# rmcar17/SpectralClusterSupertree

Hardware: AMD Instinct MI355X
Metric: top-level PCG build + Fiedler solve wall-time (s) at N taxa, 1/2/4/8 MI355X (lower is better)
Workload: dtype f64 (loop operator: fp32 image of W; fp64 renewal + confirmation)

## Files before the change

### spectralclustersupertree_amd/csrc/scs_build.hip

```cpp

#include <algorithm>

#include "scs_internal.h"

typedef unsigned long long u64;
typedef unsigned int u32;

constexpr u32 DEPTH_INF = 0xFFFFFFFFu;


__device__ __forceinline__ void rmq_offsets(int m, int a, int b, int (&o)[2]) {
    const int k = 31 - __clz(b - a);
    o[0] = k * m + a;
    o[1] = k * m + b - (1 << k);
}

template <typename K>
__device__ __forceinline__ K rmq_min(const K *__restrict__ base, int m, int a, int b) {
    int o[2];
    rmq_offsets(m, a, b, o);
    const K x = base[o[0]], y = base[o[1]];
    return x < y ? x : y;
}

// ... 391 lines not shown
};

struct ev_pair {
    hipEvent_t a = nullptr, b = nullptr;
    ~ev_pair() {
        if (a) hipEventDestroy(a);
        if (b) hipEventDestroy(b);
    }
    int init() {
        SCS_HIP_CHECK(hipEventCreate(&a));
        SCS_HIP_CHECK(hipEventCreate(&b));
        return SCS_OK;
    }
};

int levels_for(int64_t m) {
    int l = 0;
    while (((int64_t)1 << l) <= m) ++l;
    return l;
}

}

static int graph_alloc(scs_ctx *ctx, int32_t n, int32_t row_begin, int32_t row_end,
                       hipStream_t stream, scs_graph **out, int32_t col0 = 0) {
    auto *g = new scs_graph();
    g->n = n;
    g->row_begin = row_begin;
    g->row_end = row_end;
    g->col0 = col0;
    g->upper = col0 > 0 || false;
    g->ld = scs_round_up(n - col0, SCS_LD_ALIGN);
    const size_t rows = (size_t)(row_end - row_begin);
    size_t bytes = rows * (size_t)g->ld * sizeof(double);
    if (bytes < 16) bytes = 16;
    {
        const int rc = scs_block_alloc(ctx, bytes, (void **)&g->d_w);
        if (rc != SCS_OK) {
            delete g;
            return rc;
        }
        g->w_bytes = bytes;
        g->w_block = true;
    }
    if (g->ld > n - col0) {
        hipError_t e = hipMemset2DAsync(g->d_w + (n - col0), (size_t)g->ld * 8, 0,
                                        (size_t)(g->ld - (n - col0)) * 8, rows, stream);
        if (e != hipSuccess) {
            if (g->w_block) scs_block_release(ctx, g->d_w);
            else scs_dev_free(g->d_w);
            delete g;
            scs_set_error("cannot clear the padding of W: %s", hipGetErrorString(e));
            return SCS_EHIP;
        }
    }
    *out = g;
    return SCS_OK;
}

extern "C" int scs_graph_free(scs_ctx *ctx, scs_graph *g) {
    if (!g) return SCS_OK;
    if (ctx) hipSetDevice(ctx->device);
    if (g->mf) {
        if (ctx) hipStreamSynchronize(ctx->stream);
        scs_matfree_release(g);
    }
    if (ctx && g->d_w && g->w_block) {
        scs_block_release(ctx, g->d_w);
    } else if (ctx && g->d_w) {
        if (!ctx->w_cache || g->w_bytes >= ctx->w_cache_bytes) {
// ... 141 lines not shown
            k_block_records_wide<PIPE_NG><<<grid_r, 64, 0, s>>>(tb->d_tree_off, b.t0, tl0, b.nb, b.pos, b.npad, b.st_off, st,
                                                          b.am_off, b.am, b.row_begin, b.row_end, b.rec);
        else if (b.kind == PREP_MONO)
            k_block_records_mono<<<grid_r, 64, 0, s>>>(tb->d_tree_off, b.t0, tl0, b.nb, b.pos, b.npad, b.st_off, st,
                                                       b.am_off, b.am, b.row_begin, b.row_end, b.rec);
    } else {
        gap_entry *st = (gap_entry *)b.st;
        k_positions_pairs<<<grid_l, 256, 0, s>>>(tb->d_tree_off, tb->d_leaf_taxon, tb->d_adj_depth, tb->d_adj_val,
                                                 tb->d_tree_w, b.t0, tl0, b.pos, b.npad, b.st_off, st);
        if (fused)
            k_sparse_levels_fused<gap_entry><<<(unsigned)np, 1024, 0, s>>>(tb->d_tree_off, b.t0, tl0, b.st_off, st,
                                                                           b.am_off, b.am, pick_shallower_pair{});
        else
            for (int k = 1; k < max_levels; ++k)
                k_sparse_level<gap_entry><<<grid_l, 256, 0, s>>>(tb->d_tree_off, b.t0, tl0, k, b.st_off, st, b.am_off,
                                                                 b.am, pick_shallower_pair{});
        k_block_records_gen<<<grid_r, 64, 0, s>>>(tb->d_tree_off, b.t0, tl0, b.nb, b.pos, b.npad, b.st_off, st, b.am_off,
                                                  b.am, b.row_begin, b.row_end, b.rec);
    }
    SCS_HIP_CHECK(hipGetLastError());
    return SCS_OK;
}

struct pinned_ref {
    scs_ctx *ctx;
    hipStream_t stream;
    void *p = nullptr;
    bool in_flight = false;
    pinned_ref(scs_ctx *c, hipStream_t s) : ctx(c), stream(s) {}
    ~pinned_ref() {
        if (!p) return;
        if (in_flight) hipStreamSynchronize(stream);
        scs_pinned_release(ctx, p);
    }
};

}

extern "C" int scs_pcg_build(scs_ctx *ctx, const scs_tables *tb, int32_t row_begin,
                             int32_t row_end, int32_t flags, scs_graph **out,
                             scs_build_stats *stats) {
    SCS_REQUIRE(ctx && tb && out, "scs_pcg_build: null argument");
    SCS_REQUIRE((flags & ~(SCS_BUILD_MONOTONE | SCS_BUILD_SHARED | SCS_BUILD_UPPER | SCS_BUILD_SCATTER)) == 0,
                "scs_pcg_build: unknown flag bits 0x%x", flags);
    const bool scatter = (flags & SCS_BUILD_SCATTER) != 0;
    if (scatter && tb) SCS_TRY(scs_tables_finish(ctx, tb));
// ... 19 lines not shown
    static_assert(MONO_TCW == SCS_TCW, "one tile width for all kernels");
    const size_t entry_bytes = monotone ? 8 : sizeof(gap_entry);
    size_t rec_bytes = monotone ? R3_BYTES : G3_BYTES;
    const int n_cgroups = (n + cols_per_tile - 1) / cols_per_tile;
    const int64_t npad = scs_round_up((int64_t)n_cgroups * cols_per_tile, SCS_NPAD);
    bool shared = (flags & SCS_BUILD_SHARED) != 0 && world > 1;
    if (shared) {
        const int64_t nb_all = (n + SCS_TR - 1) / SCS_TR;
        const double tile_bytes = 0.5 * (double)nb_all * n_cgroups * SCS_TR * cols_per_tile * 8.0;
        if (tile_bytes * (1.0 + 1.0 / world) > 96.0 * 1024 * 1024 * 1024) shared = false;
    }
    const int b_row_begin = shared ? 0 : row_begin, b_row_end = shared ? n : row_end;
    const bool sym = !shared && (row_begin == 0 && row_end == n && world == 1);
    const bool trapezoid = (flags & SCS_BUILD_UPPER) != 0;
    if (trapezoid)
        SCS_REQUIRE(row_begin % cols_per_tile == 0,
                    "scs_pcg_build: SCS_BUILD_UPPER needs row_begin (%d) to be a multiple of %d", row_begin,
                    cols_per_tile);
    const bool upper = sym || shared || trapezoid;
    const int gb0 = b_row_begin / SCS_TR;
    const int rows = row_end - row_begin;
    const int n_blocks = (b_row_end - b_row_begin + SCS_TR - 1) / SCS_TR;

    scs_graph *g = nullptr;
    SCS_TRY(graph_alloc(ctx, n, row_begin, row_end, s, &g, trapezoid ? row_begin : 0));
    g->upper = trapezoid;
    if (scatter) SCS_HIP_CHECK(hipMemsetAsync(g->d_w, 0, (size_t)rows * (size_t)g->ld * 8, s));
    double *w_base = g->d_w - g->col0;
    struct guard {
        scs_ctx *c;
        scs_graph *g;
        ~guard() {
            if (g) scs_graph_free(c, g);
        }
    } gd{ctx, g};

    std::vector<int2> tiles;
    tiles.reserve((size_t)n_blocks * n_cgroups);
    for (int b = 0; b < n_blocks; ++b)
        for (int c = 0; c < n_cgroups; ++c) {
            if (upper && (int64_t)(c + 1) * cols_per_tile <= (int64_t)(gb0 + b) * SCS_TR) continue;
            tiles.push_back(make_int2(b, c));
        }
    {
        const bool per_xcd = !(scs_dbg("SCS_TILE_ORDER") && atoi(scs_dbg("SCS_TILE_ORDER")) == 0);
        auto xcd_reorder = [](std::vector<int2> &v) {
            if (v.size() <= 8) return;
            std::vector<int2> per[8];
            for (const int2 &t : v) per[t.x & 7].push_back(t);
            std::vector<int2> ordered;
            ordered.reserve(v.size());
            size_t at[8] = {0, 0, 0, 0, 0, 0, 0, 0};
            while (ordered.size() < v.size())
                for (int x = 0; x < 8; ++x)
                    if (at[x] < per[x].size()) ordered.push_back(per[x][at[x]++]);
            v.swap(ordered);
        };
        if (per_xcd && !shared) {
            xcd_reorder(tiles);
        } else if (per_xcd) {
            std::vector<std::vector<int2>> share(world);
            for (size_t i = 0; i < tiles.size(); ++i) share[i % world].push_back(tiles[i]);
            for (auto &v : share) xcd_reorder(v);
            for (int r = 0; r < world; ++r)
                for (size_t k = 0; k < share[r].size(); ++k) tiles[(size_t)world * k + r] = share[r][k];
        }
    }
    std::vector<int2> all_tiles;
    dev_buf d_all_tiles(ctx);
    cached_buf d_tile_out(ctx), d_gathered(ctx);
    size_t chunk_doubles = 0;
    const bool exchange_allgather =
        scs_dbg("SCS_EXCHANGE") && std::string(scs_dbg("SCS_EXCHANGE")) == "allgather";
    if (shared) {
        all_tiles.swap(tiles);
        for (size_t i = rank; i < all_tiles.size(); i += world) tiles.push_back(all_tiles[i]);
        const size_t slots = (all_tiles.size() + world - 1) / world;
        chunk_doubles = slots * SCS_TR * cols_per_tile;
        SCS_TRY(d_all_tiles.alloc(all_tiles.size() * sizeof(int2)));
        SCS_HIP_CHECK(hipMemcpyAsync(d_all_tiles.p, all_tiles.data(),
                                     all_tiles.size() * sizeof(int2), hipMemcpyHostToDevice, s));
        SCS_TRY(d_tile_out.alloc(chunk_doubles * 8));
        if (exchange_allgather) SCS_TRY(d_gathered.alloc(chunk_doubles * 8 * world));
        if (tiles.size() < slots)
            SCS_HIP_CHECK(hipMemsetAsync((double *)d_tile_out.p + (slots - 1) * SCS_TR * cols_per_tile,
                                         0, (size_t)SCS_TR * cols_per_tile * 8, s));
    }
    pooled_buf d_tiles(ctx, 0);
    SCS_TRY(d_tiles.alloc(std::max<size_t>(tiles.size(), 1) * sizeof(int2)));
    SCS_HIP_CHECK(hipMemcpyAsync(d_tiles.p, tiles.data(), tiles.size() * sizeof(int2),
                                 hipMemcpyHostToDevice, s));

    bool tree_par = sym && !scatter && !tiles.empty() && tiles.size() <= 24 && tb->n_trees >= 128;
    if (const char *e = scs_dbg("SCS_TREE_PARALLEL")) tree_par = sym && !scatter && !tiles.empty() && atoi(e) != 0;
    const size_t cells_per_tree = tiles.size() * (size_t)SCS_TR * cols_per_tile * 8;

    const size_t wide_min_tiles = 13;
    bool listed = monotone && !scatter && !tiles.empty() && tb->n_trees > 0 &&
                  (double)tb->n_leaves / ((double)tb->n_trees * std::max(n, 1)) < 1.0 / 64.0;
    if (const char *e = scs_dbg("SCS_TILE_LISTS")) listed = monotone && !scatter && !tiles.empty() && atoi(e) != 0;
    if (listed) tree_par = false;
    int wide_mode = (monotone && !scatter && !tree_par && !listed && tiles.size() >= wide_min_tiles) ? 3 : 0;
    bool wide_forced = false;
    if (const char *e = scs_dbg("SCS_WIDE")) {
        wide_mode = (monotone && !scatter && !tiles.empty() && atoi(e)) ? 3 : 0;
        wide_forced = wide_mode != 0;
        if (wide_mode) listed = false;
    }
    if (wide_mode && ctx->max_lds_bytes < (int)spec_layout::LDS_BYTES) {
        wide_mode = 0;
        wide_forced = false;
    }
    if (wide_mode) tree_par = false;
    const bool wide = wide_mode != 0;
    const int group_tiles = PIPE_NG;
    std::vector<int4> groups;
    dev_buf d_groups(ctx);
    if (wide) {
        rec_bytes = wide_layout<PIPE_NG>::BYTES;
        std::vector<std::vector<int>> of_block((size_t)n_blocks);
        for (size_t i = 0; i < tiles.size(); ++i) of_block[(size_t)tiles[i].x].push_back((int)i);
        std::vector<int4> per[8];
        for (int b = 0; b < n_blocks; ++b) {
            const std::vector<int> &v = of_block[(size_t)b];
            for (size_t k = 0; k < v.size(); k += group_tiles)
                per[b & 7].push_back(make_int4(v[k], k + 1 < v.size() ? v[k + 1] : -1,
                                               (group_tiles > 2 && k + 2 < v.size()) ? v[k + 2] : -1, 0));
        }
        size_t total = 0, at[8] = {0, 0, 0, 0, 0, 0, 0, 0};
        for (auto &v : per) total += v.size();
        groups.reserve(total);
        while (groups.size() < total)
            for (int x = 0; x < 8; ++x)
                if (at[x] < per[x].size()) groups.push_back(per[x][at[x]++]);
        SCS_TRY(d_groups.alloc(groups.size() * sizeof(int4)));
        SCS_HIP_CHECK(hipMemcpyAsync(d_groups.p, groups.data(), groups.size() * sizeof(int4),
                                     hipMemcpyHostToDevice, s));
    }

    const int M = tb->n_trees;
    std::vector<int> batch_start{0};
    {
        const int batch_trees_env = scs_dbg("SCS_BATCH_TREES") ? atoi(scs_dbg("SCS_BATCH_TREES")) : 0;
        int max_batch_trees = 256;
        {
            const double avg_leaves = (double)tb->n_leaves / std::max(M, 1);
            const double table_bytes =
                (double)table_entries((int64_t)std::max(avg_leaves - 1.0, 1.0)) * (double)entry_bytes;
            max_batch_trees = (int)std::min(256.0, std::max(64.0, 600e6 / std::max(table_bytes, 1.0)));
        }
        if (n <= 2048) max_batch_trees = 4096;
        const int arrived = tb->late_start.empty() ? M : tb->late_start[0];
        if (wide) {
            const int rest = M - (arrived < M ? arrived : 0);
            const int k = std::max(1, (rest + 511) / 512);
            max_batch_trees = std::max(96, (rest + k - 1) / k);
        }
        if (tree_par)
            max_batch_trees = (int)std::max<size_t>(16, std::min<size_t>((size_t)max_batch_trees,
                                                                         SCS_SCRATCH_KEEP / cells_per_tree));
        if (batch_trees_env > 0) max_batch_trees = batch_trees_env;
        if (tree_par)
            max_batch_trees = (int)std::max<size_t>(1, std::min<size_t>((size_t)max_batch_trees,
                                                                        SCS_SCRATCH_KEEP / std::max<size_t>(cells_per_tree, 1)));
        size_t used = 0;
        for (int t = 0; t < M; ++t) {
            const int64_t nt = tb->h_tree_off[t + 1] - tb->h_tree_off[t];
            const int64_t m = nt - 1;
            const size_t need = (size_t)table_entries(m) * entry_bytes + (size_t)argmin_entries(m) * sizeof(argmin_t) +
                                (size_t)npad * 4 + (size_t)n_blocks * rec_bytes;
            if ((used + need > ctx->ws_limit || t - batch_start.back() >= max_batch_trees ||
                 (t == arrived && batch_start.size() == 1)) &&
                t > batch_start.back()) {
                batch_start.push_back(t);
                used = 0;
            }
            used += need;
        }
        batch_start.push_back(M);
    }
    const int n_batches = (int)batch_start.size() - 1;

    struct ev_ref {
        hipEvent_t a, b;
    } ev_total, ev_prep, ev_acc;
    for (auto &e : ctx->build_events)
        if (!e) SCS_HIP_CHECK(hipEventCreate(&e));
    ev_total = {ctx->build_events[0], ctx->build_events[1]};
    ev_prep = {ctx->build_events[2], ctx->build_events[3]};
    ev_acc = {ctx->build_events[4], ctx->build_events[5]};
    float prep_ms = 0.f, acc_ms = 0.f;
    SCS_HIP_CHECK(hipEventRecord(ev_total.a, s));

    int spec_batches = 0, spec_trees = 0;
    float spec_ms = 0.f;
    bool single_batch_spec = false;
    pooled_buf d_pos(ctx, 1), d_am(ctx, 2), d_st(ctx, 3), d_stoff(ctx, 4), d_rec(ctx, 5), d_cells(ctx, 6);
    dev_buf d_pcol(ctx), d_lists(ctx), d_list_cnt(ctx);
    int listed_batches = 0;
    std::vector<size_t> off_at((size_t)n_batches + 1, 0);
    for (int bi = 0; bi < n_batches; ++bi)
        off_at[bi + 1] = off_at[bi] + 2 * (size_t)(batch_start[bi + 1] - batch_start[bi] + 1);
    pinned_ref h_off(ctx, s);
    SCS_TRY(scs_pinned_get(ctx, std::max<size_t>(off_at[n_batches], 2) * 8, &h_off.p));
    {
        int64_t *h = (int64_t *)h_off.p;
        for (int bi = 0; bi < n_batches; ++bi) {
            const int t0 = batch_start[bi], nb = batch_start[bi + 1] - t0;
            int64_t *st_off = h + off_at[bi], *am_off = st_off + nb + 1;
            st_off[0] = am_off[0] = 0;
            for (int t = 0; t < nb; ++t) {
                const int64_t m = tb->h_tree_off[t0 + t + 1] - tb->h_tree_off[t0 + t] - 1;
                st_off[t + 1] = st_off[t] + table_entries(m);
                am_off[t + 1] = am_off[t] + argmin_entries(m);
            }
        }
        SCS_TRY(d_stoff.alloc(off_at[n_batches] * 8));
        h_off.in_flight = true;
        SCS_HIP_CHECK(hipMemcpyAsync(d_stoff.p, h, off_at[n_batches] * 8, hipMemcpyHostToDevice, s));
    }
    const bool by_arrival = !(scs_dbg("SCS_PREP_BY_ARRIVAL") && atoi(scs_dbg("SCS_PREP_BY_ARRIVAL")) == 0);
    int prep_pieces = 0;
    for (int bi = 0; bi < n_batches; ++bi) {
        const int t0 = batch_start[bi], t1 = batch_start[bi + 1];
        const int nb = t1 - t0;
        const int64_t *h_st_off = (const int64_t *)h_off.p + off_at[bi], *h_am_off = h_st_off + nb + 1;
        int64_t max_n = 0;
        for (int t = t0; t < t1; ++t) max_n = std::max(max_n, tb->h_tree_off[t + 1] - tb->h_tree_off[t]);
        const size_t need_pos = (size_t)nb * npad * 4;
        const size_t need_st = (size_t)h_st_off[nb] * entry_bytes + 64;
        const size_t need_am = (size_t)h_am_off[nb] * sizeof(argmin_t) + 64;
        const size_t need_rec = (size_t)n_blocks * nb * rec_bytes;
        const int wide_min_trees = wide_forced ? 1 : 96;
        const bool wide_b = wide && (nb >= wide_min_trees || (groups.size() >= 8 * 256 && nb >= 16));
        if (wide_b) {
            ++spec_batches;
            spec_trees += nb;
            single_batch_spec = true;
        }
        SCS_TRY(d_pos.alloc(need_pos));
        SCS_TRY(d_st.alloc(need_st));
        SCS_TRY(d_am.alloc(need_am));
        SCS_TRY(d_rec.alloc(need_rec));

        SCS_HIP_CHECK(hipEventRecord(ev_prep.a, s));
        SCS_HIP_CHECK(hipMemsetAsync(d_pos.p, 0xFF, need_pos, s));
        prep_batch pb;
        pb.tb = tb;
        pb.t0 = t0;
        pb.nb = nb;
        pb.kind = !monotone ? PREP_GEN : wide_b ? PREP_WIDE : scatter ? PREP_NO_RECORDS : PREP_MONO;
        pb.pos = (int32_t *)d_pos.p;
        pb.npad = npad;
        pb.st_off = (const int64_t *)d_stoff.p + off_at[bi];
        pb.am_off = pb.st_off + nb + 1;
        pb.st = d_st.p;
        pb.am = (argmin_t *)d_am.p;
        pb.rec = (unsigned char *)d_rec.p;
        pb.n_blocks = n_blocks;
        pb.row_begin = b_row_begin;
        pb.row_end = b_row_end;
        for (int p0 = t0; p0 < t1;) {
            int p1 = t1;
            if (by_arrival)
                for (const int32_t c : tb->late_start)
                    if (c > p0 && c < p1) p1 = c;
            SCS_TRY(scs_tables_wait(ctx, tb, p1, s));
            SCS_TRY(prep_piece(pb, p0 - t0, p1 - p0, s));
            ++prep_pieces;
            p0 = p1;
        }
        SCS_HIP_CHECK(hipEventRecord(ev_prep.b, s));

        SCS_HIP_CHECK(hipEventRecord(ev_acc.a, s));
        const unsigned nt = (unsigned)tiles.size();
        if (scatter) {
            const int64_t nbk = (max_n + 63) / 64;
            k_scatter_atomic<<<dim3((unsigned)(nbk * (nbk + 1) / 2), (unsigned)nb), 256, 0, s>>>(
                tb->d_tree_off, tb->d_leaf_taxon, t0, pb.st_off, (const double *)d_st.p,
                g->d_w, g->ld);
        } else if (monotone) {
            mono_params mp;
            mp.tiles = (const int2 *)d_tiles.p;
            mp.rec = (const unsigned char *)d_rec.p;
            mp.pos = (const int32_t *)d_pos.p;
            mp.npad = npad;
            mp.stv = (const double *)d_st.p;
            mp.n_batch = nb;
            mp.w = w_base;
            mp.ld = g->ld;
            mp.n = n;
            mp.row_begin = b_row_begin;
            mp.row_end = b_row_end;
            mp.load_w = bi > 0;
            mp.mirror = (sym && bi == n_batches - 1) ? 1 : 0;
            mp.tile_out = shared ? (double *)d_tile_out.p : nullptr;
            mp.stamps = nullptr;
            mp.split_tiles = 0;
            mp.lists = nullptr;
            mp.list_cnt = nullptr;
            const bool stamp = scs_dbg("SCS_ACC_STAMP") && atoi(scs_dbg("SCS_ACC_STAMP"));
            if (wide_b) {
                wide_params wp;
                wp.m = mp;
                wp.groups = (const int4 *)d_groups.p;
                wp.producer_prio = 2;
                const unsigned ng = (unsigned)groups.size();
                dev_buf d_st8(ctx);
                if (stamp) {
                    SCS_TRY(d_st8.alloc(64));
                    SCS_HIP_CHECK(hipMemsetAsync(d_st8.p, 0, 64, s));
                    wp.m.stamps = (unsigned long long *)d_st8.p;
                }
#define SCS_LAUNCH_SPEC(SYM_, STAMP_)                                                                   \
    do {                                                                                                \
        SCS_HIP_CHECK(hipFuncSetAttribute((const void *)k_accumulate_spec<SYM_, STAMP_>,                \
                                          hipFuncAttributeMaxDynamicSharedMemorySize,                   \
                                          (int)spec_layout::LDS_BYTES));                                \
        k_accumulate_spec<SYM_, STAMP_><<<ng, spec_layout::THREADS, spec_layout::LDS_BYTES, s>>>(wp);   \
    } while (0)
                if (ng) {
                    if (stamp && sym) SCS_LAUNCH_SPEC(true, true);
                    else if (stamp) SCS_LAUNCH_SPEC(false, true);
                    else if (sym) SCS_LAUNCH_SPEC(true, false);
                    else SCS_LAUNCH_SPEC(false, false);
                }
#undef SCS_LAUNCH_SPEC
                if (stamp) {
// ... 21 lines not shown
                const char *nm[7] = {"wait loads+record", "barrier A", "combine", "search + issue",
                                     "expand", "barrier B", "cells"};
                double tot = 0;
                for (int i = 0; i < 7; ++i) tot += (double)h[i];
                for (int i = 0; i < 7; ++i)
                    fprintf(stderr, "[stamp] %-24s %6.2f %%  (%.0f cycles per wave-step)\n", nm[i],
                            100.0 * h[i] / tot, (double)h[i] / ((double)h[7] * nb));
            } else if (nt && tree_par) {
                SCS_TRY(d_cells.alloc((size_t)nb * cells_per_tree));
                mono_params ap = mp;
                ap.split_tiles = (int)nt;
                ap.load_w = 0;
                ap.mirror = 0;
                ap.tile_out = (double *)d_cells.p;
                k_accumulate_mono<true, false><<<nt * (unsigned)nb, MONO_TCW, 0, s>>>(ap);
                k_sum_tree_tiles<true, mono_params><<<nt * SCS_TR, MONO_TCW, 0, s>>>(mp, (const double *)d_cells.p,
                                                                                    (int)nt);
            } else if (nt && listed) {
                SCS_TRY(d_pcol.alloc((size_t)n_cgroups * nb));
                SCS_TRY(d_lists.alloc((size_t)nt * nb * 4));
                SCS_TRY(d_list_cnt.alloc((size_t)nt * 4));
                k_col_presence<<<dim3((unsigned)n_cgroups, (unsigned)nb), 64, 0, s>>>(
                    (const int32_t *)d_pos.p, npad, n, cols_per_tile, nb, (unsigned char *)d_pcol.p);
                k_tile_lists<<<(nt + 255) / 256, 256, 0, s>>>((const int2 *)d_tiles.p, (int)nt,
                                                             (const unsigned char *)d_rec.p, R3_BYTES, R3_CNT, nb,
                                                             (const unsigned char *)d_pcol.p, (int32_t *)d_lists.p,
                                                             (int32_t *)d_list_cnt.p);
                mp.lists = (const int32_t *)d_lists.p;
                mp.list_cnt = (const int32_t *)d_list_cnt.p;
                if (sym) k_accumulate_mono<true, false, true><<<nt, MONO_TCW, 0, s>>>(mp);
                else k_accumulate_mono<false, false, true><<<nt, MONO_TCW, 0, s>>>(mp);
                ++listed_batches;
            } else if (nt) {
                if (sym) k_accumulate_mono<true, false><<<nt, MONO_TCW, 0, s>>>(mp);
                else k_accumulate_mono<false, false><<<nt, MONO_TCW, 0, s>>>(mp);
            }
        } else {
            gen_params gp;
            gp.tiles = (const int2 *)d_tiles.p;
            gp.rec = (const unsigned char *)d_rec.p;
            gp.pos = (const int32_t *)d_pos.p;
            gp.npad = npad;
            gp.ste = (const gap_entry *)d_st.p;
            gp.n_batch = nb;
            gp.w = w_base;
            gp.ld = g->ld;
            gp.n = n;
            gp.row_begin = b_row_begin;
            gp.row_end = b_row_end;
            gp.load_w = bi > 0;
            gp.mirror = (sym && bi == n_batches - 1) ? 1 : 0;
            gp.tile_out = shared ? (double *)d_tile_out.p : nullptr;
            gp.split_tiles = 0;
            if (nt && tree_par) {
                SCS_TRY(d_cells.alloc((size_t)nb * cells_per_tree));
                gen_params ap = gp;
                ap.split_tiles = (int)nt;
                ap.load_w = 0;
                ap.mirror = 0;
                ap.tile_out = (double *)d_cells.p;
                k_accumulate_gen<true><<<nt * (unsigned)nb, MONO_TCW, 0, s>>>(ap);
                k_sum_tree_tiles<true, gen_params><<<nt * SCS_TR, MONO_TCW, 0, s>>>(gp, (const double *)d_cells.p,
                                                                                   (int)nt);
            } else if (nt) {
                if (sym) k_accumulate_gen<true><<<nt, MONO_TCW, 0, s>>>(gp);
                else k_accumulate_gen<false><<<nt, MONO_TCW, 0, s>>>(gp);
            }
        }
        SCS_HIP_CHECK(hipGetLastError());
        SCS_HIP_CHECK(hipEventRecord(ev_acc.b, s));
        if (n_batches > 1) {
            SCS_HIP_CHECK(hipEventSynchronize(ev_acc.b));
            float ms = 0.f;
            SCS_HIP_CHECK(hipEventElapsedTime(&ms, ev_prep.a, ev_prep.b));
            prep_ms += ms;
            SCS_HIP_CHECK(hipEventElapsedTime(&ms, ev_acc.a, ev_acc.b));
            acc_ms += ms;
            if (wide_b) spec_ms += ms;
        }
    }
    float exch_ms = 0.f;
    double exch_bytes = 0.0;
    if (shared && exchange_allgather) {
        ev_pair ev_x;
        SCS_TRY(ev_x.init());
        SCS_HIP_CHECK(hipEventRecord(ev_x.a, s));
        SCS_TRY(scs_comm_allgather_f64(&ctx->comm, (const double *)d_tile_out.p,
                                       (double *)d_gathered.p, chunk_doubles, s));
        k_unpack_tiles<<<(unsigned)all_tiles.size(), cols_per_tile, 0, s>>>(
            (const double *)d_gathered.p, (const int2 *)d_all_tiles.p, world,
            (int64_t)chunk_doubles, n, row_begin, row_end, g->d_w, g->ld);
        SCS_HIP_CHECK(hipGetLastError());
        SCS_HIP_CHECK(hipEventRecord(ev_x.b, s));
        SCS_HIP_CHECK(hipEventSynchronize(ev_x.b));
        SCS_HIP_CHECK(hipEventElapsedTime(&exch_ms, ev_x.a, ev_x.b));
        exch_bytes = (double)chunk_doubles * 8.0 * (world - 1);
    } else if (shared) {
        std::vector<int32_t> splits;
        SCS_TRY(scs_gather_row_splits(ctx, row_begin, row_end, n, splits));
        auto needs = [&](int dst, const int2 &t) {
            const int64_t lo = splits[dst], hi = splits[dst + 1];
            const int64_t r_lo = (int64_t)t.x * SCS_TR, r_hi = std::min<int64_t>(r_lo + SCS_TR, n);
            const int64_t c_lo = (int64_t)t.y * cols_per_tile, c_hi = std::min<int64_t>(c_lo + cols_per_tile, n);
            return (r_lo < hi && lo < r_hi) || (c_lo < hi && lo < c_hi);
        };
        std::vector<int64_t> send_off(world + 1, 0), recv_off(world + 1, 0);
        std::vector<int32_t> send_slots;
        std::vector<int2> recv_tiles;
        for (int p = 0; p < world; ++p) {
            for (size_t i = rank; i < all_tiles.size(); i += world)
                if (needs(p, all_tiles[i])) send_slots.push_back((int32_t)(i / world));
            send_off[p + 1] = (int64_t)send_slots.size() * SCS_TR * cols_per_tile;
            for (size_t i = p; i < all_tiles.size(); i += world)
// ... 15 lines not shown
                                     hipMemcpyHostToDevice, s));
        if (!send_slots.empty())
            k_pack_tiles<<<(unsigned)send_slots.size(), 256, 0, s>>>(
                (const double *)d_tile_out.p, (const int32_t *)d_slots.p, cols_per_tile, (double *)d_send.p);
        SCS_HIP_CHECK(hipGetLastError());
        SCS_TRY(scs_comm_alltoallv_f64(&ctx->comm, (const double *)d_send.p, send_off.data(),
                                       (double *)d_recv.p, recv_off.data(), s));
        if (!recv_tiles.empty())
            k_unpack_received<<<(unsigned)recv_tiles.size(), cols_per_tile, 0, s>>>(
                (const double *)d_recv.p, (const int2 *)d_rtiles.p, n, row_begin, row_end, g->d_w,
                g->ld);
        SCS_HIP_CHECK(hipGetLastError());
        SCS_HIP_CHECK(hipEventRecord(ev_x.b, s));
        SCS_HIP_CHECK(hipEventSynchronize(ev_x.b));
        SCS_HIP_CHECK(hipEventElapsedTime(&exch_ms, ev_x.a, ev_x.b));
        exch_bytes = (double)(recv_off[world] - (recv_off[rank + 1] - recv_off[rank])) * 8.0;
    }
    SCS_HIP_CHECK(hipEventRecord(ev_total.b, s));
    SCS_HIP_CHECK(hipEventSynchronize(ev_total.b));
    h_off.in_flight = false;
    SCS_TRY(scs_tables_finish(ctx, tb));
    float total_ms = 0.f;
    SCS_HIP_CHECK(hipEventElapsedTime(&total_ms, ev_total.a, ev_total.b));
    if (n_batches == 1) {
        SCS_HIP_CHECK(hipEventElapsedTime(&prep_ms, ev_prep.a, ev_prep.b));
        SCS_HIP_CHECK(hipEventElapsedTime(&acc_ms, ev_acc.a, ev_acc.b));
        if (single_batch_spec) spec_ms = acc_ms;
    }

    if (stats) {
        memset(stats, 0, sizeof(*stats));
        stats->n_taxa = n;
        stats->n_trees = M;
        stats->row_begin = row_begin;
        stats->row_end = row_end;
        stats->symmetric = shared ? 2 : (sym ? 1 : 0);
        stats->exchange_ms = exch_ms;
        stats->exchange_bytes = exch_bytes;
        stats->n_tiles = (int32_t)tiles.size();
        stats->n_batches = n_batches;
        stats->spec_batches = spec_batches;
        stats->tree_parallel_batches = tree_par ? n_batches : 0;
        stats->spec_trees = spec_trees;
        stats->listed_batches = listed_batches;
        stats->prep_pieces = prep_pieces;
        stats->spec_ms = spec_ms;
        stats->cell_trees = (double)tiles.size() * SCS_TR * cols_per_tile * (double)M;
        stats->prep_ms = prep_ms;
        stats->accumulate_ms = acc_ms;
        stats->total_ms = total_ms;
// ... 343 lines not shown
```

### spectralclustersupertree_amd/csrc/scs_ctx.hip

```cpp

#include <dlfcn.h>

#include <atomic>
#include <condition_variable>
#include <mutex>

#include "scs_internal.h"
#include "scs_arena.h"

#include <chrono>
#include <pthread.h>

#include <algorithm>
#include <cmath>

static thread_local std::string g_last_error;

void scs_set_error(const char *fmt, ...) {
    char buf[1024];
    va_list ap;
    va_start(ap, fmt);
    vsnprintf(buf, sizeof(buf), fmt, ap);
    va_end(ap);
    g_last_error = buf;
// ... 1070 lines not shown
    t->max_leaves = (int32_t)max_leaves;
    t->h_tree_off.assign(tree_off, tree_off + n_trees + 1);
    t->d_block = block;
    char *base = (char *)block;
    t->d_tree_off = (int64_t *)(base + o_off);
    t->d_leaf_taxon = (int32_t *)(base + o_tax);
    t->d_adj_depth = (int32_t *)(base + o_dep);
    t->d_adj_val = (double *)(base + o_val);
    t->d_tree_w = (double *)(base + o_w);
    unsigned *d_flags = (unsigned *)(base + o_flag);
    t->d_flags = d_flags;
    hipStream_t s = ctx->stream;
    int32_t first = n_trees, chunk = n_trees;
    if (n_taxa > 2048 && (size_t)L * 16 >= ((size_t)8 << 20) && scs_is_pinned(leaf_taxon) &&
        scs_is_pinned(adj_depth) && scs_is_pinned(adj_val)) {
        const double avg = std::max((double)L / n_trees - 1.0, 1.0);
        const double table_bytes = (std::floor(std::log2(avg)) + 1.0) * avg * 8.0;
        const int32_t per = (int32_t)std::min(256.0, std::max(64.0, 600e6 / table_bytes));
        if (n_trees >= 2 * per || n_trees - per >= 32) {
            first = std::min(per, 64);
            chunk = per;
        }
    }
    const int64_t L0 = tree_off[first];
    hipError_t e = hipMemsetAsync(d_flags, 0, 4, s);
    if (e == hipSuccess) e = hipMemcpyAsync(t->d_tree_off, tree_off, ((size_t)n_trees + 1) * 8, hipMemcpyHostToDevice, s);
    if (e == hipSuccess && L0) e = hipMemcpyAsync(t->d_leaf_taxon, leaf_taxon, (size_t)L0 * 4, hipMemcpyHostToDevice, s);
    if (e == hipSuccess && L0) e = hipMemcpyAsync(t->d_adj_depth, adj_depth, (size_t)L0 * 4, hipMemcpyHostToDevice, s);
    if (e == hipSuccess && L0) e = hipMemcpyAsync(t->d_adj_val, adj_val, (size_t)L0 * 8, hipMemcpyHostToDevice, s);
    if (e == hipSuccess) e = hipMemcpyAsync(t->d_tree_w, tree_w, (size_t)n_trees * 8, hipMemcpyHostToDevice, s);
    if (e == hipSuccess) {
        const int grid = (int)std::min<int64_t>((L0 + 255) / 256 + 1, 4096);
        k_validate_tables<<<grid, 256, 0, s>>>(t->d_leaf_taxon, t->d_adj_depth, L0, n_taxa, d_flags);
        e = hipGetLastError();
    }
    if (e == hipSuccess) e = hipMemcpyAsync(ctx->h_flags, d_flags, 4, hipMemcpyDeviceToHost, s);
    if (e == hipSuccess) e = hipStreamSynchronize(s);
    if (e == hipSuccess && first < n_trees) {
        if (!ctx->copy_stream) e = hipStreamCreateWithFlags(&ctx->copy_stream, hipStreamNonBlocking);
        hipStream_t cs = ctx->copy_stream;
        for (int32_t a = first; a < n_trees && e == hipSuccess; a += chunk) {
            const int32_t b = std::min(n_trees, a + chunk);
            const int64_t p0 = tree_off[a], cnt = tree_off[b] - tree_off[a];
            e = hipMemcpyAsync(t->d_leaf_taxon + p0, leaf_taxon + p0, (size_t)cnt * 4, hipMemcpyHostToDevice, cs);
            if (e == hipSuccess) e = hipMemcpyAsync(t->d_adj_depth + p0, adj_depth + p0, (size_t)cnt * 4, hipMemcpyHostToDevice, cs);
            if (e == hipSuccess) e = hipMemcpyAsync(t->d_adj_val + p0, adj_val + p0, (size_t)cnt * 8, hipMemcpyHostToDevice, cs);
            hipEvent_t ev = nullptr;
            if (e == hipSuccess) e = hipEventCreateWithFlags(&ev, hipEventDisableTiming);
            if (e == hipSuccess) e = hipEventRecord(ev, cs);
            if (e == hipSuccess) {
                t->late_start.push_back(a);
                t->late_ev.push_back(ev);
            } else if (ev) {
                hipEventDestroy(ev);
            }
            if (e == hipSuccess) {
                const int grid = (int)std::min<int64_t>((cnt + 255) / 256 + 1, 4096);
                k_validate_tables<<<grid, 256, 0, cs>>>(t->d_leaf_taxon + p0, t->d_adj_depth + p0, cnt, n_taxa, d_flags);
                e = hipGetLastError();
            }
        }
    }
    if (e != hipSuccess) {
        scs_tables_free(ctx, t);
        scs_set_error("table upload failed: %s", hipGetErrorString(e));
        return e == hipErrorOutOfMemory ? SCS_ENOMEM : SCS_EHIP;
    }
    const unsigned bad = *ctx->h_flags;
    if (bad) {
        scs_tables_free(ctx, t);
        scs_set_error("scs_tables_upload: %s", (bad & 1u) ? "a leaf_taxon entry is out of range [0, n_taxa)"
                                                          : "an adj_depth entry is negative");
        return SCS_EINVAL;
    }
    *out = t;
    return SCS_OK;
}
```

### spectralclustersupertree_amd/csrc/scs_internal.h

```cpp
#pragma once

#include <hip/hip_runtime.h>

#include <cstdarg>
#include <cstdint>
#include <cstdio>
#include <cstring>
#include <mutex>
#include <string>
#include <vector>

#include "../../include/scs_hip.h"

void scs_set_error(const char *fmt, ...);

#define SCS_HIP_CHECK(expr)                                                                  \
    do {                                                                                     \
        hipError_t e_ = (expr);                                                              \
        if (e_ != hipSuccess) {                                                              \
            scs_set_error("%s failed: %s (%s:%d)", #expr, hipGetErrorString(e_), __FILE__,   \
                          __LINE__);                                                         \
            return (e_ == hipErrorOutOfMemory) ? SCS_ENOMEM : SCS_EHIP;                      \
        }                                                                                    \
    } while (0)
// ... 17 lines not shown
    static const bool on = [] {
        const char *e = getenv("SCS_DEBUG");
        return e && atoi(e) != 0;
    }();
    return on ? getenv(name) : nullptr;
}

struct scs_ctx;
hipError_t scs_dev_malloc_impl(scs_ctx *ctx, void **p, size_t bytes);
hipError_t scs_dev_free(void *p);
template <typename T>
static inline hipError_t scs_dev_malloc(scs_ctx *ctx, T **p, size_t bytes) {
    return scs_dev_malloc_impl(ctx, (void **)p, bytes);
}
size_t scs_arena_free_bytes(int device);

constexpr int SCS_TR = 64;
constexpr int SCS_TCW = 256;
constexpr int SCS_NPAD = 512;
constexpr int SCS_LD_ALIGN = 512;

constexpr size_t SCS_SCRATCH_KEEP = (size_t)1 << 30;
constexpr size_t SCS_PINNED_KEEP = (size_t)2 << 30;

struct scs_ctx;
int scs_block_alloc(scs_ctx *ctx, size_t bytes, void **out);
void scs_block_release(scs_ctx *ctx, void *p);
void scs_block_drop_free(scs_ctx *ctx);
int scs_pinned_get(scs_ctx *ctx, size_t bytes, void **out);
void scs_pinned_release(scs_ctx *ctx, void *p);

struct scs_local_group;

struct scs_comm {
    int rank = 0;
    int world = 1;
    int kind = 0;
    void *rccl_comm = nullptr;
    scs_local_group *group = nullptr;
};

int scs_comm_allgather_f64(scs_comm *comm, const double *sendbuf, double *recvbuf, size_t count,
                           hipStream_t stream);
int scs_comm_alltoallv_f64(scs_comm *comm, const double *sendbuf, const int64_t *send_off,
                           double *recvbuf, const int64_t *recv_off, hipStream_t stream);
int scs_comm_init_rccl(scs_comm *comm, int rank, int world, const void *uid);
// ... 40 lines not shown
        size_t o_to = 0, o_lt = 0, o_ad = 0, o_av = 0, o_tw = 0;
        int64_t n_toff = 0, n_leaf = 0, n_tree = 0;
        unsigned char *scratch = nullptr;
        size_t scratch_cap = 0;
    };
    std::vector<small_slot> small_slots;
    hipStream_t small_stream = nullptr;
};

struct scs_tables {
    int32_t n_taxa = 0;
    int32_t n_trees = 0;
    int64_t n_leaves = 0;
    int32_t max_leaves = 0;
    std::vector<int64_t> h_tree_off;
    void *d_block = nullptr;
    int64_t *d_tree_off = nullptr;
    int32_t *d_leaf_taxon = nullptr;
    int32_t *d_adj_depth = nullptr;
    double *d_adj_val = nullptr;
    double *d_tree_w = nullptr;
    mutable std::vector<int32_t> late_start;
    mutable std::vector<hipEvent_t> late_ev;
    unsigned *d_flags = nullptr;
};

int scs_tables_wait(scs_ctx *ctx, const scs_tables *t, int32_t t_end, hipStream_t stream);
int scs_tables_finish(scs_ctx *ctx, const scs_tables *t);

struct mf_data {
    const scs_tables *tb = nullptr;
    int64_t *d_stack_off = nullptr;
    int64_t stack_total = 0;
    int b_cap = 0;
    int chunks = 1;
    double *st_val = nullptr, *st_sum = nullptr;
    int32_t *st_dep = nullptr;
    double *sm_val = nullptr, *sm_sum = nullptr, *cy_pa = nullptr, *cy_ps = nullptr;
    int32_t *sm_dep = nullptr, *cy_dep = nullptr, *sm_cnt = nullptr, *sm_root = nullptr, *cy_cnt = nullptr;
    double *x = nullptr;
    double *y = nullptr;
    double *slabs = nullptr;
    int slabs_b = 0;
    int64_t n_apply = 0;
    std::vector<int32_t> maxd;
};
// ... 72 lines not shown
```

Baseline: 0.01385.

## Cut host-side sync and setup overhead in PCG build and table upload

Several host-overhead changes go in together. The tile, group and offset arrays are packed into one pinned block and sent in a single copy. The per-batch hipEventSynchronize is dropped in favour of per-batch event pairs that are read only at the end. W allocation moves after host planning, and its 2D pad memset becomes a small kernel. Table upload now sends a small first piece and streams the rest on the copy stream without a blocking sync, validating it in one pass. The aim is to remove host stalls and extra API calls; it adds more events, more complex upload ordering, and a later validation error report.

```diff
diff --git a/spectralclustersupertree_amd/csrc/scs_build.hip b/spectralclustersupertree_amd/csrc/scs_build.hip
--- a/spectralclustersupertree_amd/csrc/scs_build.hip
+++ b/spectralclustersupertree_amd/csrc/scs_build.hip
@@ -1,5 +1,6 @@
 
 #include <algorithm>
+#include <chrono>
 
 #include "scs_internal.h"
 
@@ -437,6 +438,14 @@
 
 }
 
+__global__ __launch_bounds__(256) void k_zero_pads(double *__restrict__ w, int64_t ld, int used, int padw,
+                                                   int64_t rows) {
+    const int64_t i = (int64_t)blockIdx.x * 256 + threadIdx.x;
+    if (i >= rows * padw) return;
+    const int64_t r = i / padw;
+    w[r * ld + used + (int)(i - r * padw)] = 0.0;
+}
+
 static int graph_alloc(scs_ctx *ctx, int32_t n, int32_t row_begin, int32_t row_end,
                        hipStream_t stream, scs_graph **out, int32_t col0 = 0) {
     auto *g = new scs_graph();
@@ -458,9 +467,11 @@
         g->w_bytes = bytes;
         g->w_block = true;
     }
-    if (g->ld > n - col0) {
-        hipError_t e = hipMemset2DAsync(g->d_w + (n - col0), (size_t)g->ld * 8, 0,
-                                        (size_t)(g->ld - (n - col0)) * 8, rows, stream);
+    if (g->ld > n - col0 && rows > 0) {
+        const int padw = (int)(g->ld - (n - col0));
+        const int64_t cells = (int64_t)rows * padw;
+        k_zero_pads<<<(unsigned)((cells + 255) / 256), 256, 0, stream>>>(g->d_w, g->ld, n - col0, padw, (int64_t)rows);
+        hipError_t e = hipGetLastError();
         if (e != hipSuccess) {
             if (g->w_block) scs_block_release(ctx, g->d_w);
             else scs_dev_free(g->d_w);
@@ -648,6 +659,25 @@
     return SCS_OK;
 }
 
+template <typename T, typename KEY>
+void deal_to_xcds(std::vector<T> &v, KEY key) {
+    size_t start[9] = {0, 0, 0, 0, 0, 0, 0, 0, 0};
+    for (const T &t : v) ++start[key(t) + 1];
+    size_t longest = 0;
+    for (int x = 0; x < 8; ++x) {
+        longest = std::max(longest, start[x + 1]);
+        start[x + 1] += start[x];
+    }
+    std::vector<T> sorted(v.size());
+    size_t at[8];
+    for (int x = 0; x < 8; ++x) at[x] = start[x];
+    for (const T &t : v) sorted[at[key(t)]++] = t;
+    size_t o = 0;
+    for (size_t r = 0; r < longest; ++r)
+        for (int x = 0; x < 8; ++x)
+            if (start[x] + r < start[x + 1]) v[o++] = sorted[start[x] + r];
+}
+
 struct pinned_ref {
     scs_ctx *ctx;
     hipStream_t stream;
@@ -713,18 +743,12 @@
     const int rows = row_end - row_begin;
     const int n_blocks = (b_row_end - b_row_begin + SCS_TR - 1) / SCS_TR;
 
-    scs_graph *g = nullptr;
-    SCS_TRY(graph_alloc(ctx, n, row_begin, row_end, s, &g, trapezoid ? row_begin : 0));
-    g->upper = trapezoid;
-    if (scatter) SCS_HIP_CHECK(hipMemsetAsync(g->d_w, 0, (size_t)rows * (size_t)g->ld * 8, s));
-    double *w_base = g->d_w - g->col0;
-    struct guard {
-        scs_ctx *c;
-        scs_graph *g;
-        ~guard() {
-            if (g) scs_graph_free(c, g);
-        }
-    } gd{ctx, g};
+    const bool stamps_on = scs_dbg("SCS_BUILD_STAMPS") && atoi(scs_dbg("SCS_BUILD_STAMPS"));
+    std::vector<std::pair<const char *, std::chrono::steady_clock::time_point>> host_stamps;
+    auto host_stamp = [&](const char *what) {
+        if (stamps_on) host_stamps.emplace_back(what, std::chrono::steady_clock::now());
+    };
+    host_stamp("entry");
 
     std::vector<int2> tiles;
     tiles.reserve((size_t)n_blocks * n_cgroups);
@@ -737,15 +761,7 @@
         const bool per_xcd = !(scs_dbg("SCS_TILE_ORDER") && atoi(scs_dbg("SCS_TILE_ORDER")) == 0);
         auto xcd_reorder = [](std::vector<int2> &v) {
             if (v.size() <= 8) return;
-            std::vector<int2> per[8];
-            for (const int2 &t : v) per[t.x & 7].push_back(t);
-            std::vector<int2> ordered;
-            ordered.reserve(v.size());
-            size_t at[8] = {0, 0, 0, 0, 0, 0, 0, 0};
-            while (ordered.size() < v.size())
-                for (int x = 0; x < 8; ++x)
-                    if (at[x] < per[x].size()) ordered.push_back(per[x][at[x]++]);
-            v.swap(ordered);
+            deal_to_xcds(v, [](const int2 &t) { return t.x & 7; });
         };
         if (per_xcd && !shared) {
             xcd_reorder(tiles);
@@ -758,8 +774,8 @@
         }
     }
     std::vector<int2> all_tiles;
-    dev_buf d_all_tiles(ctx);
     cached_buf d_tile_out(ctx), d_gathered(ctx);
+    bool clear_last_slot = false;
     size_t chunk_doubles = 0;
     const bool exchange_allgather =
         scs_dbg("SCS_EXCHANGE") && std::string(scs_dbg("SCS_EXCHANGE")) == "allgather";
@@ -768,19 +784,10 @@
         for (size_t i = rank; i < all_tiles.size(); i += world) tiles.push_back(all_tiles[i]);
         const size_t slots = (all_tiles.size() + world - 1) / world;
         chunk_doubles = slots * SCS_TR * cols_per_tile;
-        SCS_TRY(d_all_tiles.alloc(all_tiles.size() * sizeof(int2)));
-        SCS_HIP_CHECK(hipMemcpyAsync(d_all_tiles.p, all_tiles.data(),
-                                     all_tiles.size() * sizeof(int2), hipMemcpyHostToDevice, s));
         SCS_TRY(d_tile_out.alloc(chunk_doubles * 8));
         if (exchange_allgather) SCS_TRY(d_gathered.alloc(chunk_doubles * 8 * world));
-        if (tiles.size() < slots)
-            SCS_HIP_CHECK(hipMemsetAsync((double *)d_tile_out.p + (slots - 1) * SCS_TR * cols_per_tile,
-                                         0, (size_t)SCS_TR * cols_per_tile * 8, s));
-    }
-    pooled_buf d_tiles(ctx, 0);
-    SCS_TRY(d_tiles.alloc(std::max<size_t>(tiles.size(), 1) * sizeof(int2)));
-    SCS_HIP_CHECK(hipMemcpyAsync(d_tiles.p, tiles.data(), tiles.size() * sizeof(int2),
-                                 hipMemcpyHostToDevice, s));
+        clear_last_slot = tiles.size() < slots;
+    }
 
     bool tree_par = sym && !scatter && !tiles.empty() && tiles.size() <= 24 && tb->n_trees >= 128;
     if (const char *e = scs_dbg("SCS_TREE_PARALLEL")) tree_par = sym && !scatter && !tiles.empty() && atoi(e) != 0;
@@ -806,28 +813,28 @@
     const bool wide = wide_mode != 0;
     const int group_tiles = PIPE_NG;
     std::vector<int4> groups;
-    dev_buf d_groups(ctx);
     if (wide) {
         rec_bytes = wide_layout<PIPE_NG>::BYTES;
-        std::vector<std::vector<int>> of_block((size_t)n_blocks);
-        for (size_t i = 0; i < tiles.size(); ++i) of_block[(size_t)tiles[i].x].push_back((int)i);
-        std::vector<int4> per[8];
+        std::vector<size_t> of_start((size_t)n_blocks + 1, 0);
+        for (const int2 &t : tiles) ++of_start[(size_t)t.x + 1];
+        for (int b = 0; b < n_blocks; ++b) of_start[(size_t)b + 1] += of_start[(size_t)b];
+        std::vector<int> of_tile(tiles.size());
+        {
+            std::vector<size_t> at(of_start.begin(), of_start.end() - 1);
+            for (size_t i = 0; i < tiles.size(); ++i) of_tile[at[(size_t)tiles[i].x]++] = (int)i;
+        }
+        groups.reserve(tiles.size() / group_tiles + (size_t)n_blocks);
         for (int b = 0; b < n_blocks; ++b) {
-            const std::vector<int> &v = of_block[(size_t)b];
-            for (size_t k = 0; k < v.size(); k += group_tiles)
-                per[b & 7].push_back(make_int4(v[k], k + 1 < v.size() ? v[k + 1] : -1,
-                                               (group_tiles > 2 && k + 2 < v.size()) ? v[k + 2] : -1, 0));
-        }
-        size_t total = 0, at[8] = {0, 0, 0, 0, 0, 0, 0, 0};
-        for (auto &v : per) total += v.size();
-        groups.reserve(total);
-        while (groups.size() < total)
-            for (int x = 0; x < 8; ++x)
-                if (at[x] < per[x].size()) groups.push_back(per[x][at[x]++]);
-        SCS_TRY(d_groups.alloc(groups.size() * sizeof(int4)));
-        SCS_HIP_CHECK(hipMemcpyAsync(d_groups.p, groups.data(), groups.size() * sizeof(int4),
-                                     hipMemcpyHostToDevice, s));
-    }
+            const int *v = of_tile.data() + of_start[(size_t)b];
+            const size_t nv = of_start[(size_t)b + 1] - of_start[(size_t)b];
+            for (size_t k = 0; k < nv; k += group_tiles)
+                groups.push_back(make_int4(v[k], k + 1 < nv ? v[k + 1] : -1,
+                                           (group_tiles > 2 && k + 2 < nv) ? v[k + 2] : -1, b));
+        }
+        deal_to_xcds(groups, [](const int4 &g4) { return g4.w & 7; });
+        for (int4 &g4 : groups) g4.w = 0;
+    }
+    host_stamp("tile list and groups");
 
     const int M = tb->n_trees;
     std::vector<int> batch_start{0};
@@ -841,7 +848,7 @@
             max_batch_trees = (int)std::min(256.0, std::max(64.0, 600e6 / std::max(table_bytes, 1.0)));
         }
         if (n <= 2048) max_batch_trees = 4096;
-        const int arrived = tb->late_start.empty() ? M : tb->late_start[0];
+        const int arrived = tb->late_start.empty() ? M : std::min<int>(M, std::max<int>(tb->first_batch, tb->late_start[0]));
         if (wide) {
             const int rest = M - (arrived < M ? arrived : 0);
             const int k = std::max(1, (rest + 511) / 512);
@@ -874,28 +881,53 @@
 
     struct ev_ref {
         hipEvent_t a, b;
-    } ev_total, ev_prep, ev_acc;
+    } ev_total;
     for (auto &e : ctx->build_events)
         if (!e) SCS_HIP_CHECK(hipEventCreate(&e));
     ev_total = {ctx->build_events[0], ctx->build_events[1]};
-    ev_prep = {ctx->build_events[2], ctx->build_events[3]};
-    ev_acc = {ctx->build_events[4], ctx->build_events[5]};
+    struct batch_events {
+        scs_ctx *c;
+        std::vector<hipEvent_t> ev;
+        std::vector<char> is_spec;
+        ~batch_events() {
+            for (size_t i = 4; i < ev.size(); ++i) c->event_pool.push_back(ev[i]);
+        }
+    } bev{ctx, {}, {}};
+    bev.ev.assign(ctx->build_events + 2, ctx->build_events + 6);
+    bev.ev.reserve(4 * (size_t)n_batches);
+    while (bev.ev.size() < 4 * (size_t)n_batches) {
+        hipEvent_t e = nullptr;
+        if (!ctx->event_pool.empty()) {
+            e = ctx->event_pool.back();
+            ctx->event_pool.pop_back();
+        } else {
+            SCS_HIP_CHECK(hipEventCreate(&e));
+        }
+        bev.ev.push_back(e);
+    }
+    bev.is_spec.assign((size_t)n_batches, 0);
     float prep_ms = 0.f, acc_ms = 0.f;
-    SCS_HIP_CHECK(hipEventRecord(ev_total.a, s));
 
     int spec_batches = 0, spec_trees = 0;
     float spec_ms = 0.f;
-    bool single_batch_spec = false;
     pooled_buf d_pos(ctx, 1), d_am(ctx, 2), d_st(ctx, 3), d_stoff(ctx, 4), d_rec(ctx, 5), d_cells(ctx, 6);
     dev_buf d_pcol(ctx), d_lists(ctx), d_list_cnt(ctx);
     int listed_batches = 0;
     std::vector<size_t> off_at((size_t)n_batches + 1, 0);
     for (int bi = 0; bi < n_batches; ++bi)
         off_at[bi + 1] = off_at[bi] + 2 * (size_t)(batch_start[bi + 1] - batch_start[bi] + 1);
+    auto up256 = [](size_t b) { return (b + 255) / 256 * 256; };
+    const size_t o_tiles = up256(std::max<size_t>(off_at[n_batches], 2) * 8);
+    const size_t o_groups = o_tiles + up256(std::max<size_t>(tiles.size(), 1) * sizeof(int2));
+    const size_t o_all = o_groups + up256(groups.size() * sizeof(int4));
+    const size_t setup_bytes = o_all + up256(all_tiles.size() * sizeof(int2));
     pinned_ref h_off(ctx, s);
-    SCS_TRY(scs_pinned_get(ctx, std::max<size_t>(off_at[n_batches], 2) * 8, &h_off.p));
+    SCS_TRY(scs_pinned_get(ctx, setup_bytes, &h_off.p));
     {
         int64_t *h = (int64_t *)h_off.p;
+        if (!tiles.empty()) memcpy((char *)h_off.p + o_tiles, tiles.data(), tiles.size() * sizeof(int2));
+        if (!groups.empty()) memcpy((char *)h_off.p + o_groups, groups.data(), groups.size() * sizeof(int4));
+        if (!all_tiles.empty()) memcpy((char *)h_off.p + o_all, all_tiles.data(), all_tiles.size() * sizeof(int2));
         for (int bi = 0; bi < n_batches; ++bi) {
             const int t0 = batch_start[bi], nb = batch_start[bi + 1] - t0;
             int64_t *st_off = h + off_at[bi], *am_off = st_off + nb + 1;
@@ -906,11 +938,38 @@
                 am_off[t + 1] = am_off[t] + argmin_entries(m);
             }
         }
-        SCS_TRY(d_stoff.alloc(off_at[n_batches] * 8));
-        h_off.in_flight = true;
-        SCS_HIP_CHECK(hipMemcpyAsync(d_stoff.p, h, off_at[n_batches] * 8, hipMemcpyHostToDevice, s));
-    }
+    }
+    host_stamp("batch plan, offsets, set-up block");
+
+    scs_graph *g = nullptr;
+    SCS_TRY(graph_alloc(ctx, n, row_begin, row_end, s, &g, trapezoid ? row_begin : 0));
+    g->upper = trapezoid;
+    struct guard {
+        scs_ctx *c;
+        scs_graph *g;
+        ~guard() {
+            if (g) scs_graph_free(c, g);
+        }
+    } gd{ctx, g};
+    host_stamp("W block and its padding kernel");
+    if (scatter) SCS_HIP_CHECK(hipMemsetAsync(g->d_w, 0, (size_t)rows * (size_t)g->ld * 8, s));
+    double *w_base = g->d_w - g->col0;
+    if (clear_last_slot) {
+        const size_t slots = (all_tiles.size() + world - 1) / world;
+        SCS_HIP_CHECK(hipMemsetAsync((double *)d_tile_out.p + (slots - 1) * SCS_TR * cols_per_tile, 0,
+                                     (size_t)SCS_TR * cols_per_tile * 8, s));
+    }
+    SCS_HIP_CHECK(hipEventRecord(ev_total.a, s));
+    SCS_TRY(d_stoff.alloc(setup_bytes));
+    h_off.in_flight = true;
+    SCS_HIP_CHECK(hipMemcpyAsync(d_stoff.p, h_off.p, setup_bytes, hipMemcpyHostToDevice, s));
+    const int2 *d_tiles = (const int2 *)((const char *)d_stoff.p + o_tiles);
+    const int4 *d_groups = (const int4 *)((const char *)d_stoff.p + o_groups);
+    const int2 *d_all_tiles = (const int2 *)((const char *)d_stoff.p + o_all);
+    host_stamp("set-up copy queued");
     const bool by_arrival = !(scs_dbg("SCS_PREP_BY_ARRIVAL") && atoi(scs_dbg("SCS_PREP_BY_ARRIVAL")) == 0);
+    const bool cut_first_piece = scs_dbg("SCS_PREP_FIRST_PIECE") && atoi(scs_dbg("SCS_PREP_FIRST_PIECE"));
+    const int32_t no_cut_below = (tb->late_start.empty() || cut_first_piece) ? 0 : tb->first_batch;
     int prep_pieces = 0;
     for (int bi = 0; bi < n_batches; ++bi) {
         const int t0 = batch_start[bi], t1 = batch_start[bi + 1];
@@ -927,13 +986,15 @@
         if (wide_b) {
             ++spec_batches;
             spec_trees += nb;
-            single_batch_spec = true;
         }
         SCS_TRY(d_pos.alloc(need_pos));
         SCS_TRY(d_st.alloc(need_st));
         SCS_TRY(d_am.alloc(need_am));
         SCS_TRY(d_rec.alloc(need_rec));
 
+        const ev_ref ev_prep{bev.ev[4 * (size_t)bi], bev.ev[4 * (size_t)bi + 1]};
+        const ev_ref ev_acc{bev.ev[4 * (size_t)bi + 2], bev.ev[4 * (size_t)bi + 3]};
+        bev.is_spec[(size_t)bi] = wide_b;
         SCS_HIP_CHECK(hipEventRecord(ev_prep.a, s));
         SCS_HIP_CHECK(hipMemsetAsync(d_pos.p, 0xFF, need_pos, s));
         prep_batch pb;
@@ -955,7 +1016,7 @@
             int p1 = t1;
             if (by_arrival)
                 for (const int32_t c : tb->late_start)
-                    if (c > p0 && c < p1) p1 = c;
+                    if (c > p0 && c < p1 && c >= no_cut_below) p1 = c;
             SCS_TRY(scs_tables_wait(ctx, tb, p1, s));
             SCS_TRY(prep_piece(pb, p0 - t0, p1 - p0, s));
             ++prep_pieces;
@@ -972,7 +1033,7 @@
                 g->d_w, g->ld);
         } else if (monotone) {
             mono_params mp;
-            mp.tiles = (const int2 *)d_tiles.p;
+            mp.tiles = d_tiles;
             mp.rec = (const unsigned char *)d_rec.p;
             mp.pos = (const int32_t *)d_pos.p;
             mp.npad = npad;
@@ -994,7 +1055,7 @@
             if (wide_b) {
                 wide_params wp;
                 wp.m = mp;
-                wp.groups = (const int4 *)d_groups.p;
+                wp.groups = d_groups;
                 wp.producer_prio = 2;
                 const unsigned ng = (unsigned)groups.size();
                 dev_buf d_st8(ctx);
@@ -1062,7 +1123,7 @@
                 SCS_TRY(d_list_cnt.alloc((size_t)nt * 4));
                 k_col_presence<<<dim3((unsigned)n_cgroups, (unsigned)nb), 64, 0, s>>>(
                     (const int32_t *)d_pos.p, npad, n, cols_per_tile, nb, (unsigned char *)d_pcol.p);
-                k_tile_lists<<<(nt + 255) / 256, 256, 0, s>>>((const int2 *)d_tiles.p, (int)nt,
+                k_tile_lists<<<(nt + 255) / 256, 256, 0, s>>>(d_tiles, (int)nt,
                                                              (const unsigned char *)d_rec.p, R3_BYTES, R3_CNT, nb,
                                                              (const unsigned char *)d_pcol.p, (int32_t *)d_lists.p,
                                                              (int32_t *)d_list_cnt.p);
@@ -1077,7 +1138,7 @@
             }
         } else {
             gen_params gp;
-            gp.tiles = (const int2 *)d_tiles.p;
+            gp.tiles = d_tiles;
             gp.rec = (const unsigned char *)d_rec.p;
             gp.pos = (const int32_t *)d_pos.p;
             gp.npad = npad;
@@ -1109,15 +1170,9 @@
         }
         SCS_HIP_CHECK(hipGetLastError());
         SCS_HIP_CHECK(hipEventRecord(ev_acc.b, s));
-        if (n_batches > 1) {
+        if (n_batches > 1 && scs_dbg("SCS_BATCH_EVENT_WAIT") && atoi(scs_dbg("SCS_BATCH_EVENT_WAIT")))
             SCS_HIP_CHECK(hipEventSynchronize(ev_acc.b));
-            float ms = 0.f;
-            SCS_HIP_CHECK(hipEventElapsedTime(&ms, ev_prep.a, ev_prep.b));
-            prep_ms += ms;
-            SCS_HIP_CHECK(hipEventElapsedTime(&ms, ev_acc.a, ev_acc.b));
-            acc_ms += ms;
-            if (wide_b) spec_ms += ms;
-        }
+        if (bi == 0) host_stamp("first batch queued");
     }
     float exch_ms = 0.f;
     double exch_bytes = 0.0;
@@ -1128,7 +1183,7 @@
         SCS_TRY(scs_comm_allgather_f64(&ctx->comm, (const double *)d_tile_out.p,
                                        (double *)d_gathered.p, chunk_doubles, s));
         k_unpack_tiles<<<(unsigned)all_tiles.size(), cols_per_tile, 0, s>>>(
-            (const double *)d_gathered.p, (const int2 *)d_all_tiles.p, world,
+            (const double *)d_gathered.p, d_all_tiles, world,
             (int64_t)chunk_doubles, n, row_begin, row_end, g->d_w, g->ld);
         SCS_HIP_CHECK(hipGetLastError());
         SCS_HIP_CHECK(hipEventRecord(ev_x.b, s));
@@ -1190,10 +1245,19 @@
     SCS_TRY(scs_tables_finish(ctx, tb));
     float total_ms = 0.f;
     SCS_HIP_CHECK(hipEventElapsedTime(&total_ms, ev_total.a, ev_total.b));
-    if (n_batches == 1) {
-        SCS_HIP_CHECK(hipEventElapsedTime(&prep_ms, ev_prep.a, ev_prep.b));
-        SCS_HIP_CHECK(hipEventElapsedTime(&acc_ms, ev_acc.a, ev_acc.b));
-        if (single_batch_spec) spec_ms = acc_ms;
+    for (int bi = 0; bi < n_batches; ++bi) {
+        float ms = 0.f;
+        SCS_HIP_CHECK(hipEventElapsedTime(&ms, bev.ev[4 * (size_t)bi], bev.ev[4 * (size_t)bi + 1]));
+        prep_ms += ms;
+        SCS_HIP_CHECK(hipEventElapsedTime(&ms, bev.ev[4 * (size_t)bi + 2], bev.ev[4 * (size_t)bi + 3]));
+        acc_ms += ms;
+        if (bev.is_spec[(size_t)bi]) spec_ms += ms;
+    }
+    if (stamps_on) {
+        host_stamp("final synchronisation");
+        for (size_t i = 1; i < host_stamps.size(); ++i)
+            fprintf(stderr, "[build stamps] %-40s %8.1f us\n", host_stamps[i].first,
+                    std::chrono::duration<double, std::micro>(host_stamps[i].second - host_stamps[i - 1].second).count());
     }
 
     if (stats) {
diff --git a/spectralclustersupertree_amd/csrc/scs_ctx.hip b/spectralclustersupertree_amd/csrc/scs_ctx.hip
--- a/spectralclustersupertree_amd/csrc/scs_ctx.hip
+++ b/spectralclustersupertree_amd/csrc/scs_ctx.hip
@@ -1116,25 +1116,38 @@
             chunk = per;
         }
     }
-    const int64_t L0 = tree_off[first];
-    hipError_t e = hipMemsetAsync(d_flags, 0, 4, s);
+    int32_t piece = first;
+    const bool small_piece = !(scs_dbg("SCS_FIRST_PIECE") && atoi(scs_dbg("SCS_FIRST_PIECE")) == 0);
+    if (first < n_trees && small_piece) {
+        piece = 1;
+        while (piece < first && (size_t)tree_off[piece + 1] * 16 <= SCS_FIRST_PIECE_BYTES) ++piece;
+    }
+    t->first_batch = first;
+    const int64_t L0 = tree_off[piece];
+    hipError_t e = hipMemsetAsync(d_flags, 0, 8, s);
     if (e == hipSuccess) e = hipMemcpyAsync(t->d_tree_off, tree_off, ((size_t)n_trees + 1) * 8, hipMemcpyHostToDevice, s);
     if (e == hipSuccess && L0) e = hipMemcpyAsync(t->d_leaf_taxon, leaf_taxon, (size_t)L0 * 4, hipMemcpyHostToDevice, s);
     if (e == hipSuccess && L0) e = hipMemcpyAsync(t->d_adj_depth, adj_depth, (size_t)L0 * 4, hipMemcpyHostToDevice, s);
     if (e == hipSuccess && L0) e = hipMemcpyAsync(t->d_adj_val, adj_val, (size_t)L0 * 8, hipMemcpyHostToDevice, s);
     if (e == hipSuccess) e = hipMemcpyAsync(t->d_tree_w, tree_w, (size_t)n_trees * 8, hipMemcpyHostToDevice, s);
+    hipEvent_t ev_landed = nullptr;
+    if (e == hipSuccess && piece < n_trees && small_piece) {
+        e = hipEventCreateWithFlags(&ev_landed, hipEventDisableTiming);
+        if (e == hipSuccess) e = hipEventRecord(ev_landed, s);
+    }
     if (e == hipSuccess) {
         const int grid = (int)std::min<int64_t>((L0 + 255) / 256 + 1, 4096);
-        k_validate_tables<<<grid, 256, 0, s>>>(t->d_leaf_taxon, t->d_adj_depth, L0, n_taxa, d_flags);
+        k_validate_tables<<<grid, 256, 0, s>>>(t->d_leaf_taxon, t->d_adj_depth, L0, n_taxa, d_flags + 1);
         e = hipGetLastError();
     }
-    if (e == hipSuccess) e = hipMemcpyAsync(ctx->h_flags, d_flags, 4, hipMemcpyDeviceToHost, s);
-    if (e == hipSuccess) e = hipStreamSynchronize(s);
-    if (e == hipSuccess && first < n_trees) {
+    if (e == hipSuccess) e = hipMemcpyAsync(ctx->h_flags, d_flags + 1, 4, hipMemcpyDeviceToHost, s);
+    if (e == hipSuccess && !small_piece) e = hipStreamSynchronize(s);
+    if (e == hipSuccess && piece < n_trees) {
         if (!ctx->copy_stream) e = hipStreamCreateWithFlags(&ctx->copy_stream, hipStreamNonBlocking);
         hipStream_t cs = ctx->copy_stream;
-        for (int32_t a = first; a < n_trees && e == hipSuccess; a += chunk) {
-            const int32_t b = std::min(n_trees, a + chunk);
+        if (e == hipSuccess && ev_landed) e = hipStreamWaitEvent(cs, ev_landed, 0);
+        for (int32_t a = piece; a < n_trees && e == hipSuccess;) {
+            const int32_t b = a < first ? first : std::min(n_trees, a + chunk);
             const int64_t p0 = tree_off[a], cnt = tree_off[b] - tree_off[a];
             e = hipMemcpyAsync(t->d_leaf_taxon + p0, leaf_taxon + p0, (size_t)cnt * 4, hipMemcpyHostToDevice, cs);
             if (e == hipSuccess) e = hipMemcpyAsync(t->d_adj_depth + p0, adj_depth + p0, (size_t)cnt * 4, hipMemcpyHostToDevice, cs);
@@ -1148,13 +1161,25 @@
             } else if (ev) {
                 hipEventDestroy(ev);
             }
-            if (e == hipSuccess) {
+            if (e == hipSuccess && !small_piece) {
                 const int grid = (int)std::min<int64_t>((cnt + 255) / 256 + 1, 4096);
                 k_validate_tables<<<grid, 256, 0, cs>>>(t->d_leaf_taxon + p0, t->d_adj_depth + p0, cnt, n_taxa, d_flags);
                 e = hipGetLastError();
             }
-        }
-    }
+            a = b;
+        }
+        if (e == hipSuccess && small_piece) {
+            const int64_t p0 = tree_off[piece], cnt = L - p0;
+            const int grid = (int)std::min<int64_t>((cnt + 255) / 256 + 1, 4096);
+            k_validate_tables<<<grid, 256, 0, cs>>>(t->d_leaf_taxon + p0, t->d_adj_depth + p0, cnt, n_taxa, d_flags);
+            e = hipGetLastError();
+        }
+    }
+    if (small_piece) {
+        const hipError_t w = hipStreamSynchronize(s);
+        if (e == hipSuccess) e = w;
+    }
+    if (ev_landed) hipEventDestroy(ev_landed);
     if (e != hipSuccess) {
         scs_tables_free(ctx, t);
         scs_set_error("table upload failed: %s", hipGetErrorString(e));
diff --git a/spectralclustersupertree_amd/csrc/scs_internal.h b/spectralclustersupertree_amd/csrc/scs_internal.h
--- a/spectralclustersupertree_amd/csrc/scs_internal.h
+++ b/spectralclustersupertree_amd/csrc/scs_internal.h
@@ -63,6 +63,7 @@
 
 constexpr size_t SCS_SCRATCH_KEEP = (size_t)1 << 30;
 constexpr size_t SCS_PINNED_KEEP = (size_t)2 << 30;
+constexpr size_t SCS_FIRST_PIECE_BYTES = (size_t)5 << 19;
 
 struct scs_ctx;
 int scs_block_alloc(scs_ctx *ctx, size_t bytes, void **out);
@@ -149,6 +150,7 @@
     double *d_tree_w = nullptr;
     mutable std::vector<int32_t> late_start;
     mutable std::vector<hipEvent_t> late_ev;
+    int32_t first_batch = 0;
     unsigned *d_flags = nullptr;
 };
 
```

New measurement: 0.01377 (median of 6 runs). Within noise of the previous version (-0.5%).
